# jaeyoungjo99/ELiMaLoc

Measured on AMD Instinct MI355X. Metric: ICP registrations/sec, 128k-pt scan vs 10M-pt map; pose err vs CPU ref, higher is better.
Workload: dtype f64

## Files before the change

elimaloc_amd/csrc/elm_api.cpp:

```cpp
#include <dlfcn.h>
#include <hip/hip_runtime.h>
#include <math.h>
#include <stdio.h>
#include <stdlib.h>
#include <string.h>
#include <unistd.h>

#include <algorithm>
#include <array>
#include <chrono>
#include <map>
#include <mutex>
#include <new>
#include <set>
#include <string>
#include <thread>
#include <vector>

#include "elm_hostapi.hpp"
#include "elm_internal.hpp"
#include "elm_la.hpp"

using namespace elm;

// ... 63 lines not shown
    int device = 0;
    uint64_t id = 0;
    hipStream_t stream = nullptr;
    hipStream_t copy_stream = nullptr, order_stream = nullptr, poll_stream = nullptr;
    hipEvent_t ev_iter[4] = {nullptr, nullptr, nullptr, nullptr};
    std::vector<hipEvent_t> ev_groups;
    uint16_t* d_hilbert = nullptr;
    DevBuf d_order_jobs, d_order_tmp, d_arena, d_raw, d_flagged, d_asym;
    DevBuf d_q0, d_q1, d_q2, d_q3, d_q4, d_q5;
    DevBuf d_reloc[16];
    bool work_counters = false;
    void* h_jobs = nullptr;
    size_t h_jobs_cap = 0;
    std::string last_error;
    DevBuf d_scans, d_state, d_partials, d_sums, d_T0, d_trace, d_stage_pts, d_active, d_queue, d_ds;
    int stream_hint_count = 0, stream_hint_slots = 0, stream_hint_iters = 0;
    int* h_active = nullptr;
    int iter_hint = 0;
    int iter_ring[8] = {0, 0, 0, 0, 0, 0, 0, 0};
    unsigned iter_ring_pos = 0;
    const void* iter_key_map = nullptr;
    int iter_key_method = -1, iter_key_batch = 0;
    void* h_state = nullptr;
    size_t h_state_cap = 0;
    void* h_trace = nullptr;
    size_t h_trace_cap = 0;
    void* h_stage = nullptr;
    size_t h_stage_cap = 0;
    std::vector<uint32_t> h_key, h_ord, h_tmp;
    std::vector<struct elm_scan*> scan_free;
// ... 169 lines not shown
    }
    {
        std::lock_guard<std::mutex> lk(g_live_mu);
        if (!g_live_ctx.erase(ctx)) return;
    }
    (void)hipSetDevice(ctx->device);
    if (ctx->stream) (void)hipStreamSynchronize(ctx->stream);
    if (ctx->comm && g_rccl.comm_destroy) g_rccl.comm_destroy(ctx->comm);
    for (hipStream_t st : {ctx->copy_stream, ctx->order_stream, ctx->poll_stream})
        if (st) { (void)hipStreamSynchronize(st); (void)hipStreamDestroy(st); }
    for (hipEvent_t e : {ctx->ev_iter[0], ctx->ev_iter[1], ctx->ev_iter[2], ctx->ev_iter[3]})
        if (e) (void)hipEventDestroy(e);
    for (hipEvent_t e : ctx->ev_groups) (void)hipEventDestroy(e);
    if (ctx->d_hilbert) (void)hipFree(ctx->d_hilbert);
    if (ctx->h_jobs) (void)hipHostFree(ctx->h_jobs);
    DevBuf* bufs[] = {&ctx->d_scans, &ctx->d_state, &ctx->d_partials, &ctx->d_sums, &ctx->d_T0, &ctx->d_trace, &ctx->d_stage_pts, &ctx->d_active, &ctx->d_queue, &ctx->d_ds,
                      &ctx->d_order_jobs, &ctx->d_order_tmp, &ctx->d_arena, &ctx->d_raw, &ctx->d_flagged, &ctx->d_asym, &ctx->d_q0, &ctx->d_q1, &ctx->d_q2, &ctx->d_q3, &ctx->d_q4, &ctx->d_q5};
    if (ctx->h_active) (void)hipHostFree(ctx->h_active);
    for (DevBuf* b : bufs)
        if (b->p) (void)hipFree(b->p);
    for (DevBuf& b : ctx->d_reloc)
        if (b.p) (void)hipFree(b.p);
    for (auto& b : ctx->scan_pool) (void)hipFree(b.first);
    for (elm_scan* f : ctx->scan_free) delete f;
    if (ctx->h_state) (void)hipHostFree(ctx->h_state);
    if (ctx->h_trace) (void)hipHostFree(ctx->h_trace);
    if (ctx->h_stage) (void)hipHostFree(ctx->h_stage);
    if (ctx->h_desc) (void)hipHostFree(ctx->h_desc);
    for (hipEvent_t e : ctx->events) (void)hipEventDestroy(e);
    if (ctx->stream) (void)hipStreamDestroy(ctx->stream);
    delete ctx;
// ... 1922 lines not shown
        q.hd[s].blk_begin = cap_blocks * (uint32_t)s; q.hd[s].blk_end = cap_blocks * (uint32_t)(s + 1);
    }
    elm_iter_trace* d_trace = nullptr;
    if (trace && (rc = reserve_trace(ctx, count, &d_trace)) != ELM_OK) return rc;
    HIPCHK(ctx, hipMemcpyAsync(q.d_q, q.hq, q.ctrl_off + sizeof(StreamCtrl), hipMemcpyHostToDevice, ctx->stream));
    HIPCHK(ctx, hipMemcpyAsync(ctx->d_scans.p, q.hd, (size_t)S * sizeof(ScanDesc), hipMemcpyHostToDevice, ctx->stream));
    HIPCHK(ctx, hipMemsetAsync(ctx->d_active.p, 0, 2 * sizeof(int), ctx->stream));
    if ((rc = set_reg_params(ctx, cfg, pc, blocks, S, cap_blocks)) != ELM_OK) return rc;
    const RegParams& rp = ctx->rp;

    ScanState* st = (ScanState*)ctx->d_state.p;
    ScanDesc* dsc = (ScanDesc*)ctx->d_scans.p;
    int* d_active = (int*)ctx->d_active.p;
    const bool distributed = (ctx->comm != nullptr) || (ctx->hook != nullptr);
    (void)hipGetLastError();
    launch_stream_refill(ctx->stream, dsc, st, S, q.d_q, q.d_qT0, q.d_out, q.d_ctrl, 1);
    ctx->events_used = 0;
    const int hard_limit = ((count + S - 1) / S + 1) * cfg->max_iteration;
    const bool same_shape = ctx->stream_hint_count == count && ctx->stream_hint_slots == S;
    const int predicted = same_shape ? ctx->stream_hint_iters : 0;
    double* const partials = (double*)ctx->d_partials.p;
    double* const sums = (double*)ctx->d_sums.p;
    int it = 0;
    for (; it < hard_limit; ++it) {
        if ((rc = enqueue_accumulate(ctx, map, dsc, S, blocks, st, rp, pc, partials)) != ELM_OK) return rc;
        if (distributed) {
            launch_solve(ctx->stream, dsc, S, st, partials, sums, rp, d_trace, 1, d_active);
            if ((rc = exchange(ctx, sums, (size_t)S * (rp.asym ? kSums + kAsymRecord : kSums))) != ELM_OK) return rc;
            const StreamArgs sv = {dsc, q.d_q, q.d_qT0, q.d_out, q.d_ctrl, 0,  1, 0, it};
            launch_solve(ctx->stream, dsc, S, st, partials, sums, rp, d_trace, 2, d_active, &sv);
            launch_stream_refill(ctx->stream, dsc, st, S, q.d_q, q.d_qT0, q.d_out, q.d_ctrl, 0,  0);
        } else {
            const StreamArgs sa = {dsc, q.d_q, q.d_qT0, q.d_out, q.d_ctrl, 0, 0, 0, it};
            launch_solve(ctx->stream, dsc, S, st, partials, sums, rp, d_trace, 0, d_active, &sa);
        }
        const int done_iters = it + 1;
        const bool look = predicted > 0 ? done_iters >= predicted : (done_iters >= (count + S - 1) / S && (done_iters % 2) == 0);
        if (look) {
            HIPCHK(ctx, hipMemcpyAsync(ctx->h_active, &q.d_ctrl->completed, sizeof(int), hipMemcpyDeviceToHost, ctx->stream));
            HIPCHK(ctx, hipStreamSynchronize(ctx->stream));
            if (*ctx->h_active == count) { ++it; break; }
        }
    }
    if ((rc = prof_mark(ctx)) != ELM_OK) return rc;
    HIPCHK(ctx, hipGetLastError());
    HIPCHK(ctx, hipMemcpyAsync(ctx->h_state, q.d_out, (size_t)count * sizeof(ScanState), hipMemcpyDeviceToHost, ctx->stream));
    if (trace) HIPCHK(ctx, hipMemcpyAsync(ctx->h_trace, ctx->d_trace.p, trace_bytes(count), hipMemcpyDeviceToHost, ctx->stream));
    ctx->h_active[2] = 0;
// ... 843 lines not shown
```

elimaloc_amd/csrc/elm_dev_pairs.hpp:

```cpp
#pragma once
#include <float.h>
#include <hip/hip_runtime.h>

#include "elm_internal.hpp"
#include "elm_la.hpp"

namespace elm {




__device__ __forceinline__ unsigned xcd_remap(unsigned bid, unsigned nb) {
    unsigned q = nb >> 3, r = nb & 7u, xcd = bid & 7u, idx = bid >> 3;
    return (xcd < r ? xcd * (q + 1) : r * (q + 1) + (xcd - r) * q) + idx;
}

struct Probe {
    int vid;
    unsigned start, cnt;
};
__device__ __forceinline__ Probe probe_voxel(const DevMap& m, int kx, int ky, int kz) {
    unsigned h = hash3(kx, ky, kz) & m.mask;
    Probe p;
    p.vid = -1;
// ... 371 lines not shown
    if (!(dfin < rp.th2)) return;
    if (bvid < 0) bmx = bmy = bmz = 0.0;
    voxel_pair<ELM_VGICP, ASSIGN>(acc, m, S, rp, gx, gy, gz, bvid, bmx, bmy, bmz);
}

__device__ __forceinline__ int find_scan(const ScanDesc* __restrict__ scans, int batch, unsigned L, const RegParams& rp) {
    if (rp.uniform_blocks) return (int)(L / rp.uniform_blocks);
    int lo = 0, hi = batch - 1;
    while (lo < hi) {
        const int mid = (lo + hi + 1) >> 1;
        if (scans[mid].blk_begin <= L) lo = mid; else hi = mid - 1;
    }
    return lo;
}

__device__ __forceinline__ void block_reduce_store(double* acc, double (*red)[32], double* __restrict__ out) {
    const int lane = threadIdx.x & 63, wave = threadIdx.x >> 6;
#pragma unroll
    for (int k = 0; k < 32; ++k) {
        const double v = wave_sum(acc[k]);
        if (lane == 0) red[wave][k] = v;
    }
    __syncthreads();
    if (threadIdx.x < 32)
        out[threadIdx.x] = ((red[0][threadIdx.x] + red[1][threadIdx.x]) + red[2][threadIdx.x]) + red[3][threadIdx.x];
}


__device__ __forceinline__ void publish_and_reduce(double value, unsigned L, int, unsigned, unsigned, double* __restrict__ partials, const RegParams&, double*) {
    if (threadIdx.x < (unsigned)kSums) partials[(size_t)L * kSums + threadIdx.x] = value;
// ... 13 lines not shown
```

elimaloc_amd/csrc/elm_internal.hpp:

```cpp
#pragma once
#include <hip/hip_runtime.h>
#include <stdint.h>

#include "../../include/elimaloc_hip.h"

namespace elm {

struct __attribute__((aligned(32))) HashSlot {
    int32_t kx, ky, kz;
    int32_t vid;
    uint32_t start;
    uint32_t cnt;
    uint32_t pad0, pad1;
};

struct __attribute__((packed, aligned(4))) Pt3 {
    float x, y, z;
};

struct __attribute__((aligned(16))) GridBlk {
    float x[4], y[4], z[4];
};

struct __attribute__((aligned(64))) VoxRec {
// ... 108 lines not shown
    int32_t total;
    int32_t ready;
    int32_t done_iter;
};

struct StreamArgs {
    ScanDesc* scans;
    const QueueItem* queue;
    const double* qT0;
    ScanState* out_state;
    StreamCtrl* ctrl;
    int32_t hostfed;
    int32_t save_only;
    int32_t stride;
    int32_t iter;
};

struct RegParams {
    double th;
    double th2;
    double lm_lambda;
    double term_thr;
    double min_overlap;
    double max_fitness;
    int32_t method;
    int32_t max_iter;
    uint32_t uniform_blocks;
    int32_t radar;
    int32_t _reserved0;
    int32_t stats;
    uint32_t* flagged;
    int32_t rank_check;
    int32_t _pad_rc;
    double* asym;
    double* asym_sums;
    double radar_var[3];
    const double* query;
    int32_t* q_out;
};
constexpr int kAsymRecord = 16;
constexpr int kRadarRecord = 64;

constexpr int kTileShift = 3, kTile = 1 << kTileShift;
constexpr int kBlock = 256;
constexpr int kInitPack = 8;
struct InitPack {
    ScanDesc d[kInitPack];
    double T0[kInitPack][16];
};
constexpr int kSums = ELM_PACKED_SUMS;

void launch_init_state(hipStream_t s, ScanState* st, const double* T0, int batch, int map_empty, int* active);
void launch_init_pack(hipStream_t s, ScanDesc* scans, ScanState* st, const InitPack& pack, int batch, int map_empty, int* active, const unsigned* n_dev);
void launch_stream_refill(hipStream_t s, ScanDesc* scans, ScanState* st, int slots, const QueueItem* queue, const double* qT0,
                          ScanState* out_state, StreamCtrl* ctrl, int first, int save = 1);
void launch_accumulate_radar(hipStream_t s, const DevMap& m, const ScanDesc* scans, int batch, int total_blocks, ScanState* st, double* partials,
                             const RegParams& rp);
void launch_accumulate_direct(hipStream_t s, const DevMap& m, const ScanDesc* scans, int batch, int total_blocks,
                              ScanState* st, double* partials, const RegParams& rp);
void launch_solve(hipStream_t s, const ScanDesc* scans, int batch, ScanState* st, const double* partials,
                  double* sums, const RegParams& rp, elm_iter_trace* trace, int mode, int* active, const StreamArgs* refill = nullptr);
void launch_nbr_count(hipStream_t s, const DevMap& m, const int32_t* qkeys, uint32_t n_q, uint32_t* counts, uint32_t* nocc);
void launch_accumulate_vnbr(hipStream_t s, const DevMap& m, const ScanDesc* scans, int batch, int total_blocks,
                            ScanState* st, double* partials, const RegParams& rp);
void launch_vnbr_fill(hipStream_t s, const DevMap& m, const int32_t* qkeys, uint32_t n_q, const uint32_t* offsets, VoxBlk* out_blk);
void launch_vox_rec_fill(hipStream_t s, const DevMap& m, VoxRec* out);
void launch_vface(hipStream_t s, const DevMap& m, const uint32_t* offsets, const uint32_t* counts, uint32_t n_q, uint32_t* face_cnt,
                  const uint32_t* face_off, VoxRec* out, int plain);
void launch_accumulate_cell(hipStream_t s, const DevMap& m, const ScanDesc* scans, int batch, int total_blocks,
                            ScanState* st, double* partials, const RegParams& rp);
// ... 135 lines not shown
```

elimaloc_amd/csrc/elm_k_cell.hip:

```cpp
#include <float.h>
#include <algorithm>
#include <hip/hip_runtime.h>

#include "elm_internal.hpp"
#include "elm_la.hpp"
#include "elm_dev_grid.hpp"

namespace elm {

template <int METHOD>
__global__ __launch_bounds__(kBlock, (METHOD == ELM_P2P ? kCellWaves : kCellWaves - 1)) void k_accumulate_cell(const DevMap m, const ScanDesc* __restrict__ scans, int batch,
                                                                            unsigned total_blocks, const ScanState* __restrict__ st,
                                                                            double* __restrict__ partials, const RegParams rp) {
    constexpr int NV = (METHOD == ELM_P2P) ? kP2PVals : kSums;
    __shared__ double s_buf[kRedPass * kBlock];
    __shared__ double s_red[kSums];
    __shared__ int s_res[kBlock];
    __shared__ int s_tst[kBlock];
    __shared__ unsigned s_cnt[kBlock / 64];
    __shared__ double s_asym[(METHOD == ELM_GICP) ? kAsymSums : 1];
    __shared__ unsigned s_hitw[kBlock / 64];
    PairSum PA;
    pair_sum_zero(PA);
    static_assert(sizeof(HardRec) * kBlock <= sizeof(double) * kRedPass * kBlock, "HardRec queue must fit the reduction buffer");
    const unsigned L = xcd_remap(blockIdx.x, total_blocks);
    const int s = find_scan(scans, batch, L, rp);
    const ScanState& S = st[s];
    if (S.done) return;
    const ScanDesc sd = scans[s];
    if (L >= sd.blk_end) return;
    const unsigned i = (L - sd.blk_begin) * kBlock + threadIdx.x;
    const bool valid = i < sd.n;
    double v[NV];
#pragma unroll
    for (int k = 0; k < NV; ++k) v[k] = 0.0;
    double px = 0.0, py = 0.0, pz = 0.0, gx = 0.0, gy = 0.0, gz = 0.0;
    QProbe qp;
    qp.start = 0; qp.cnt = 0; qp.nocc = 0; qp.qid = -1;
    int bj = -1;
    int n_tested = 0;
    float hr2 = __builtin_inff();
// ... 242 lines not shown
```

elimaloc_amd/csrc/elm_k_grid.hip:

```cpp
#include <float.h>
#include <algorithm>
#include <hip/hip_runtime.h>

#include "elm_internal.hpp"
#include "elm_la.hpp"
#include "elm_dev_grid.hpp"

namespace elm {

template <int METHOD, int COMPACT, int TILED, int STATS, int WIDE>
__global__ __launch_bounds__(kBlock, (METHOD == ELM_P2P ? (STATS ? 7 : kGridWaves) : kGicpWaves)) void k_accumulate_grid(
       const DevMap m, const ScanDesc* __restrict__ scans, int batch,
                                                                            unsigned total_blocks, const ScanState* __restrict__ st,
                                                                            double* __restrict__ partials, const RegParams rp) {
    constexpr int kStats = (STATS == 1) ? 1 : 0;
    constexpr bool QUERY = STATS == 2;
    constexpr int NV = (METHOD == ELM_P2P) ? (kStats ? kP2PVals : kP2PVals - 3) : kSums;
    __shared__ double s_buf[kRedPass * kBlock];
    __shared__ double s_red[kSums];
    __shared__ int s_res[kBlock];
    __shared__ int s_tst[kStats ? kBlock : 1];
    __shared__ float s_pz[METHOD == ELM_P2P ? kBlock : 1];
    __shared__ unsigned s_st[kStats ? kBlock : 1];
    __shared__ unsigned s_cnt[kBlock / 64];
    const unsigned L = xcd_remap(blockIdx.x, total_blocks);
    const int s = find_scan(scans, batch, L, rp);
    const ScanState& S = st[s];
    if (S.done) return;
    const ScanDesc sd = scans[s];
    if (L >= sd.blk_end) return;
    const unsigned i = (L - sd.blk_begin) * kBlock + threadIdx.x;
    const bool valid = i < sd.n;
    double v[(METHOD == ELM_P2P) ? NV : 1];
#pragma unroll
    for (int k = 0; k < ((METHOD == ELM_P2P) ? NV : 1); ++k) v[k] = 0.0;
    PairSum P;
    if (METHOD != ELM_P2P) pair_sum_zero(P);
    int bj = -1;
    int n_tested = 0;
    float hr2 = __builtin_inff();
    bool hard = false;
// ... 343 lines not shown
```

elimaloc_amd/csrc/elm_k_solve.hip:

```cpp
#include <float.h>
#include <algorithm>
#include <hip/hip_runtime.h>

#include "elm_internal.hpp"
#include "elm_la.hpp"
#include "elm_dev_reduce.hpp"

namespace elm {

__device__ void update_inverse(ScanState& S) {
    double R[9];
    for (int r = 0; r < 3; ++r)
        for (int c = 0; c < 3; ++c) R[r * 3 + c] = S.T[c * 4 + r];
    inv3(R, S.Rinv);
    for (int r = 0; r < 3; ++r)
        S.tinv[r] = -((S.Rinv[r * 3] * S.T[12] + S.Rinv[r * 3 + 1] * S.T[13]) + S.Rinv[r * 3 + 2] * S.T[14]);
}

__device__ void init_scan_state(ScanState& S, const double* __restrict__ T0, int reg, int map_empty) {
    for (int k = 0; k < 16; ++k) S.T[k] = T0[k];
    update_inverse(S);
    S.fitness = 0.0;
    for (int k = 0; k < 36; ++k) S.local_cov[k] = (k % 7 == 0) ? 1.0 : 0.0;
    S.n_corr_last = 0.0;
// ... 22 lines not shown
    ScanDesc d = pack.d[s];
    if (n_dev) {
        d.n = *n_dev;
        d.n_total = d.n;
        d.blk_end = d.blk_begin + (d.n + kBlock - 1) / kBlock;
    }
    scans[s] = d;
    init_scan_state(st[s], pack.T0[s], s, map_empty);
}
void launch_init_pack(hipStream_t s, ScanDesc* scans, ScanState* st, const InitPack& pack, int batch, int map_empty, int* active, const unsigned* n_dev) {
    hipLaunchKernelGGL(k_init_pack, dim3(1), dim3(64), 0, s, scans, st, pack, batch, map_empty, active, n_dev);
}

constexpr int kMaxSlots = 4096;
__global__ __launch_bounds__(1024) void k_stream_refill(ScanDesc* scans, ScanState* st, int slots, const QueueItem* __restrict__ queue,
                                                       const double* __restrict__ qT0, ScanState* out_state, StreamCtrl* ctrl, int first, int save) {
    __shared__ int s_assign[kMaxSlots];
    __shared__ int s_save[kMaxSlots];
    for (int s = threadIdx.x; s < slots; s += blockDim.x) s_save[s] = (!first && st[s].done && st[s].reg >= 0) ? st[s].reg : -1;
    __syncthreads();
    {
        __shared__ int s_wtot[16];
        const int per = (slots + (int)blockDim.x - 1) / (int)blockDim.x, s0 = (int)threadIdx.x * per, s1 = min(slots, s0 + per);
        int mine = 0;
        for (int s = s0; s < s1; ++s) mine += (first || s_save[s] >= 0) ? 1 : 0;
        int inc = mine;
#pragma unroll
        for (int off = 1; off < 64; off <<= 1) {
            const int o = __shfl_up(inc, off, 64);
            if ((int)(threadIdx.x & 63u) >= off) inc += o;
        }
// ... 28 lines not shown
        for (int k = (int)(threadIdx.x & 63); k < W; k += 64) dst[k] = src[k];
    }
    __syncthreads();
    for (int s = threadIdx.x; s < slots; s += blockDim.x) {
        const int r = s_assign[s];
        if (r >= 0) {
            const QueueItem q = queue[r];
            scans[s].pts = q.pts;
            scans[s].n = q.n;
            scans[s].n_total = q.n_total;
            init_scan_state(st[s], qT0 + (size_t)r * 16, r, 0);
        } else if (r == -2) {
            st[s].done = 1;
            st[s].reg = -1;
        }
    }
}

__device__ __forceinline__ void wave_ldlt6(double a, const double* b, double x[6], bool want_inv, double& inv_elem) {
    const int lane = threadIdx.x & 63;
    const int li = (lane < 36) ? lane / 6 : 0, lj = (lane < 36) ? lane % 6 : 0;
    unsigned active = 0x3Fu;
    int order[6];
    double piv[6];
    int rank_i = 6, rank_j = 6, rank_l = 6;
    double d0[6];
    int pos[6];
#pragma unroll
    for (int i = 0; i < 6; ++i) { d0[i] = fabs(__shfl(a, i * 7, 64)); pos[i] = i; }
    auto d0_of = [&](int r) { return r == 0 ? d0[0] : r == 1 ? d0[1] : r == 2 ? d0[2] : r == 3 ? d0[3] : r == 4 ? d0[4] : d0[5]; };
#pragma unroll
// ... 144 lines not shown
        return (r < sa.ctrl->total) ? r : -1;
    }
    if (!sa.hostfed) {
        const int r = atomicAdd(&sa.ctrl->next, 1);
        return (r < sa.ctrl->total) ? r : -1;
    }
    int old = __hip_atomic_load(&sa.ctrl->next, __ATOMIC_RELAXED, __HIP_MEMORY_SCOPE_AGENT);
    for (;;) {
        const int ready = __hip_atomic_load(&sa.ctrl->ready, __ATOMIC_RELAXED, __HIP_MEMORY_SCOPE_SYSTEM);
        if (old >= ready) return -1;
        const int seen = atomicCAS(&sa.ctrl->next, old, old + 1);
        if (seen == old) return old;
        old = seen;
    }
}
__device__ __forceinline__ void start_slot(const StreamArgs& sa, ScanState& S, int s, int prev) {
    const int lane = threadIdx.x & 63;
    int r = 0;
    if (lane == 0) r = claim_registration(sa, prev);
    r = __shfl(r, 0, 64);
    if (r >= 0) {
        const double* T0 = sa.qT0 + (size_t)r * 16;
        if (lane >= 1 && lane < 37) S.local_cov[lane - 1] = ((lane - 1) % 7 == 0) ? 1.0 : 0.0;
        if (lane == 0) {
            const QueueItem q = sa.queue[r];
            sa.scans[s].pts = q.pts;
            sa.scans[s].n = q.n;
            sa.scans[s].n_total = q.n_total;
            for (int k = 0; k < 16; ++k) S.T[k] = T0[k];
            update_inverse(S);
            S.fitness = 0.0;
            S.n_corr_last = 0.0;
            S.pt_iters = 0.0; S.cand_total = 0.0; S.occ_total = 0.0; S.fallback_blocks = 0.0; S.tested_total = 0.0;
            S.done = 0;
            S.success = 0;
            S.gate = 0;
            S.iters = 0;
            S.reg = r;
            S._pad = 0;
        }
    } else if (lane == 0) {
        S.done = 1;
        S.reg = -1;
    }
}
__device__ __forceinline__ void finish_slot(const StreamArgs& sa, ScanState& S, int s) {
#if !defined(__gfx950__) && !defined(__gfx942__) && !defined(__gfx90a__) && defined(__HIP_DEVICE_COMPILE__)
#error "finish_slot relies on gfx9 memory ordering (one vmcnt for loads and stores, write-through vector L1)"
#endif
    constexpr int W = (int)(sizeof(ScanState) / sizeof(double));
    const int lane = threadIdx.x & 63;
    __builtin_amdgcn_fence(__ATOMIC_RELEASE, "workgroup");
    __builtin_amdgcn_s_waitcnt(0);
    __builtin_amdgcn_wave_barrier();
    __builtin_amdgcn_fence(__ATOMIC_ACQUIRE, "workgroup");
    const int reg_old = __hip_atomic_load(&S.reg, __ATOMIC_RELAXED, __HIP_MEMORY_SCOPE_AGENT);
    const double* src = reinterpret_cast<const double*>(&S);
    double* dst = reinterpret_cast<double*>(&sa.out_state[reg_old]);
    for (int k = lane; k < W; k += 64) dst[k] = __hip_atomic_load(src + k, __ATOMIC_RELAXED, __HIP_MEMORY_SCOPE_AGENT);
    if (lane == 0 && atomicAdd(&sa.ctrl->completed, 1) + 1 == sa.ctrl->total) sa.ctrl->done_iter = sa.iter;
    __builtin_amdgcn_fence(__ATOMIC_RELEASE, "workgroup");
    __builtin_amdgcn_s_waitcnt(0);
    __builtin_amdgcn_wave_barrier();
    if (sa.save_only) return;
    start_slot(sa, S, s, reg_old);
}

constexpr int kSolveThreads = 1024;
__device__ __forceinline__ double rank_check_id(int reg, int iters) {
    return 16.0 * (double)((reg < 0 ? -1 : (reg & 0x7FFFF)) + 1) + (double)(iters & 15);
}
template <int NT>
__global__ __launch_bounds__(NT, 1) void k_solve(const ScanDesc* scans, ScanState* st,
                                                         const double* __restrict__ partials, double* sums,
                                                         const RegParams rp, elm_iter_trace* trace, int mode, int* active,
                                                         const StreamArgs sa) {
    const int s = blockIdx.x;
    ScanState& S = st[s];
    const int t = threadIdx.x;
    __shared__ double tot[kSums];
    __shared__ double part[kSolveThreads / 32][kSums];
    static_assert(NT == kSolveThreads, "solve workgroup size");
    const bool done = S.done != 0;
    const bool radar = rp.radar != 0;
    __shared__ double full[36];
    const bool asym = rp.asym != nullptr && !radar && rp.method != ELM_P2P;
    __shared__ double dsum[kAsymSums];
    __shared__ double apart[kSolveThreads / kAsymSums][kAsymSums];
    if (radar) {
        double a = 0.0;
        if (mode != 2) {
            const int k = t & 63, g = t >> 6;
            double* part64 = &part[0][0];
            double v = 0.0;
            if (!done) {
                const ScanDesc sd = scans[s];
                for (unsigned b = sd.blk_begin + g; b < sd.blk_end; b += kSolveThreads / 64) v += partials[(size_t)b * kRadarSums + k];
            }
            part64[g * 64 + k] = v;
            __syncthreads();
            if (t < 64) {
                a = part64[t];
#pragma unroll
                for (int q = 1; q < kSolveThreads / 64; ++q) a += part64[q * 64 + t];
                if (mode == 1) sums[(size_t)s * kRadarSums + t] = (t < kRadarAcc) ? a : 0.0;
            }
            if (mode == 1) return;
        } else if (t < 64) {
            a = sums[(size_t)s * kRadarSums + t];
        }
        if (t < 64) {
            if (t < 36) full[t] = a;
            else if (t < kRadarAcc) tot[21 + (t - 36)] = a;
        }
    } else if (mode != 2) {
        const int k = t & 31;
        constexpr unsigned G = kSolveThreads / 32;
        auto group_sum = [&](int g) -> double {
            double v = 0.0;
            if (!done) {
                const ScanDesc sd = scans[s];
                unsigned b = sd.blk_begin + g;
                double v0 = 0.0, v1 = 0.0, v2 = 0.0, v3 = 0.0;
                for (; b + 15 * G < sd.blk_end; b += 16 * G) {
                    double a[16];
#pragma unroll
                    for (int q = 0; q < 16; ++q) a[q] = partials[(size_t)(b + q * G) * kSums + k];
#pragma unroll
                    for (int q = 0; q < 16; q += 4) { v0 += a[q]; v1 += a[q + 1]; v2 += a[q + 2]; v3 += a[q + 3]; }
                }
                for (; b + 3 * G < sd.blk_end; b += 4 * G) {
                    const double a0 = partials[(size_t)b * kSums + k], a1 = partials[(size_t)(b + G) * kSums + k];
                    const double a2 = partials[(size_t)(b + 2 * G) * kSums + k], a3 = partials[(size_t)(b + 3 * G) * kSums + k];
                    v0 += a0; v1 += a1; v2 += a2; v3 += a3;
                }
                if (b < sd.blk_end) { v0 += partials[(size_t)b * kSums + k]; b += G; }
// ... 3 lines not shown
            }
            return v;
        };
        if (NT == kSolveThreads) {
            part[t >> 5][k] = group_sum(t >> 5);
        } else {
#pragma unroll 1
            for (int g = t >> 5; g < (int)G; g += NT / 32) part[g][k] = group_sum(g);
        }
        if (asym) {
            constexpr int GA = kSolveThreads / kAsymSums;
            const int k2 = t & (kAsymSums - 1);
            auto side_sum = [&](int g) -> double {
                double v = 0.0;
                if (!done) {
                    const ScanDesc sd = scans[s];
                    for (unsigned b = sd.blk_begin + (unsigned)g; b < sd.blk_end; b += (unsigned)GA) v += rp.asym[(size_t)b * kAsymSums + k2];
                }
                return v;
            };
            if (NT == kSolveThreads) {
                apart[t / kAsymSums][k2] = side_sum(t / kAsymSums);
            } else {
#pragma unroll 1
                for (int g = t / kAsymSums; g < GA; g += NT / kAsymSums) apart[g][k2] = side_sum(g);
            }
        }
        __syncthreads();
        if (t < 32) {
            double a = part[0][t];
#pragma unroll
// ... 59 lines not shown
                double row = 0.0;
                for (int l = 0; l < 3; ++l) row += hw[(bi + k) * 6 + (bj + l)] * S.T[jj * 4 + l];
                h += S.T[ii * 4 + k] * row;
            }
            if (i <= j) tot[tri(i, j)] = h;
            if (nonsym) full[t] = h;
        }
        if (t < 6) {
            const int bi = (t / 3) * 3, ii = t % 3;
            tot[21 + t] = (S.T[ii * 4 + 0] * bw[bi] + S.T[ii * 4 + 1] * bw[bi + 1]) + S.T[ii * 4 + 2] * bw[bi + 2];
        }
        __builtin_amdgcn_s_waitcnt(0);
        __builtin_amdgcn_wave_barrier();
    }

    const ScanDesc sd = scans[s];
    const int iter = S.iters + 1;
    const double n_corr = tot[28];
    if (lead) {
        S.iters = iter;
        S.n_corr_last = n_corr;
        S.pt_iters += (double)sd.n_total;
        S.cand_total += tot[29];
        S.occ_total += tot[30];
        const double fb = floor(tot[31] / 1099511627776.0);
        S.fallback_blocks += fb;
        S.tested_total += tot[31] - fb * 1099511627776.0;
    }
    elm_iter_trace* tr = (trace && iter <= ELM_MAX_ITER_TRACE) ? &trace[(size_t)S.reg * ELM_MAX_ITER_TRACE + (iter - 1)] : nullptr;

    const float ratio_f = (float)n_corr / (float)sd.n_total;
    if ((double)ratio_f < rp.min_overlap) {
        if (lead) {
            if (tr) {
                for (int k = 0; k < 36; ++k) tr->JTJ[k] = 0.0;
                for (int k = 0; k < 6; ++k) { tr->JTr[k] = 0.0; tr->x[k] = 0.0; }
                tr->residual_sum = tot[27];
                tr->n_corr = n_corr;
                tr->step_norm = 0.0;
                for (int k = 0; k < 16; ++k) tr->T[k] = S.T[k];
            }
            S.done = 1;
            atomicSub(active, 1);
            S.success = 0;
            S.gate = 2;
        }
        if (sa.ctrl) finish_slot(sa, S, s);
        return;
    }
    const double fitness = tot[27] / n_corr;

    const int li = (t < 36) ? t / 6 : 0, lj = (t < 36) ? t % 6 : 0;
    const bool full36 = radar || nonsym;
    const double hij = full36 ? full[(li < lj ? lj : li) * 6 + (li < lj ? li : lj)] : tot[tri(li < lj ? li : lj, li < lj ? lj : li)];
    const double a = (li == lj) ? hij + rp.lm_lambda * hij : hij;
    double x[6], inv_elem;
    wave_ldlt6(a, &tot[21], x, rp.method == ELM_GICP && !full36, inv_elem);
    if (rp.method == ELM_GICP && !full36 && t < 36) S.local_cov[t] = inv_elem;
    if (rp.method == ELM_GICP && full36) {
        const double el = (t < 36) ? ((li == lj) ? full[t] + rp.lm_lambda * full[t] : full[t]) : 0.0;
        const double inv_el = wave_inverse6_partial_piv(el);
        const double inv_t = __shfl(inv_el, lj * 6 + li, 64);
// ... 20 lines not shown
            for (int k = 0; k < 6; ++k) { tr->JTr[k] = tot[21 + k]; tr->x[k] = x[k]; }
            tr->residual_sum = tot[27];
            tr->n_corr = n_corr;
            tr->step_norm = step;
            for (int k = 0; k < 16; ++k) tr->T[k] = Tn[k];
        }
        if (step < rp.term_thr || iter >= rp.max_iter) {
            S.done = 1;
            atomicSub(active, 1);
            const bool bad = fitness > rp.max_fitness;
            S.success = bad ? 0 : 1;
            S.gate = bad ? 3 : 0;
            fin = true;
        }
    }
    if (sa.ctrl && __shfl((int)fin, 0, 64)) finish_slot(sa, S, s);
}

__device__ __forceinline__ void smallest_eigenvector3(const double C[9], double n[3]) {
    double A[9] = {C[0], C[3], C[6], C[3], C[4], C[7], C[6], C[7], C[8]};
    double V[9] = {1, 0, 0, 0, 1, 0, 0, 0, 1};
    for (int sweep = 0; sweep < 60; ++sweep) {
        const double off = fabs(A[3]) + fabs(A[6]) + fabs(A[7]);
        if (off == 0.0) break;
        for (int p = 0; p < 2; ++p)
            for (int q = p + 1; q < 3; ++q) {
                if (A[p * 3 + q] == 0.0) continue;
                const double theta = (A[q * 3 + q] - A[p * 3 + p]) / (2.0 * A[p * 3 + q]);
                const double t = (theta >= 0 ? 1.0 : -1.0) / (fabs(theta) + sqrt(theta * theta + 1.0));
                const double c = 1.0 / sqrt(t * t + 1.0), s = t * c;
                for (int k = 0; k < 3; ++k) { const double akp = A[k * 3 + p], akq = A[k * 3 + q]; A[k * 3 + p] = c * akp - s * akq; A[k * 3 + q] = s * akp + c * akq; }
// ... 93 lines not shown

__global__ void k_slots_idle(ScanDesc* scans, ScanState* st, int slots, unsigned cap_blocks) {
    const int s = blockIdx.x * blockDim.x + threadIdx.x;
    if (s >= slots) return;
    scans[s].pts = nullptr; scans[s].n = 0; scans[s].n_total = 0;
    scans[s].blk_begin = cap_blocks * (unsigned)s; scans[s].blk_end = cap_blocks * (unsigned)(s + 1);
    st[s].done = 1;
    st[s].reg = -1;
}

__global__ void k_publish_ready(StreamCtrl* ctrl, int ready) {
    __hip_atomic_store(&ctrl->ready, ready, __ATOMIC_RELAXED, __HIP_MEMORY_SCOPE_SYSTEM);
}

void launch_stream_refill(hipStream_t s, ScanDesc* scans, ScanState* st, int slots, const QueueItem* queue, const double* qT0,
                          ScanState* out_state, StreamCtrl* ctrl, int first, int save) {
    hipLaunchKernelGGL(k_stream_refill, dim3(1), dim3(1024), 0, s, scans, st, slots, queue, qT0, out_state, ctrl, first, save);
}

void launch_init_state(hipStream_t s, ScanState* st, const double* T0, int batch, int map_empty, int* active) {
    hipLaunchKernelGGL(k_init_state, dim3((batch + 63) / 64), dim3(64), 0, s, st, T0, batch, map_empty, active);
}

void launch_solve(hipStream_t s, const ScanDesc* scans, int batch, ScanState* st, const double* partials,
                  double* sums, const RegParams& rp, elm_iter_trace* trace, int mode, int* active, const StreamArgs* refill) {
    StreamArgs sa = {nullptr, nullptr, nullptr, nullptr, nullptr, 0, 0, 0, 0};
    if (refill) sa = *refill;
    const int threads = mode == 2 ? 64 : kSolveThreads;
    hipLaunchKernelGGL(k_solve<kSolveThreads>, dim3(batch), dim3(threads), 0, s, scans, st, partials, sums, rp, trace, mode, active, sa);
}

void launch_publish_ready(hipStream_t s, StreamCtrl* ctrl, int ready) { hipLaunchKernelGGL(k_publish_ready, dim3(1), dim3(1), 0, s, ctrl, ready); }

void launch_slots_idle(hipStream_t s, ScanDesc* scans, ScanState* st, int slots, unsigned cap_blocks) {
    hipLaunchKernelGGL(k_slots_idle, dim3((slots + 255) / 256), dim3(256), 0, s, scans, st, slots, cap_blocks);
}

int stream_max_slots() { return kMaxSlots; }

}
```

elimaloc_amd/csrc/elm_k_vnbr.hip:

```cpp
#include <float.h>
#include <algorithm>
#include <hip/hip_runtime.h>

#include "elm_internal.hpp"
#include "elm_la.hpp"
#include "elm_dev_grid.hpp"

namespace elm {


constexpr int kVnbrRecs = 3;
constexpr int kAvgRecs = 1;
constexpr int kVnbrBlks = 1;
constexpr int kVnbrWaves = 1;
template <int METHOD, int COMPACT, int STATS, int FACES>
__global__ __launch_bounds__(kBlock, kVnbrWaves) void k_accumulate_vnbr(const DevMap m, const ScanDesc* __restrict__ scans, int batch,
                                                            unsigned total_blocks, const ScanState* __restrict__ st,
                                                            double* __restrict__ partials, const RegParams rp) {
    constexpr int kStats = (STATS == 1) ? 1 : 0;
    constexpr bool QUERY = STATS == 2;
    __shared__ double s_buf[kRedPass * kBlock];
    __shared__ double s_red[kSums];
    const unsigned L = xcd_remap(blockIdx.x, total_blocks);
    const int s = find_scan(scans, batch, L, rp);
    const ScanState& S = st[s];
    if (S.done) return;
    const ScanDesc sd = scans[s];
    if (L >= sd.blk_end) return;
    const unsigned i = (L - sd.blk_begin) * kBlock + threadIdx.x;
    const bool valid = i < sd.n;
    if (FACES == 3) {
        if (rp.flagged[L] == 0u) return;
        __syncthreads();
        if (threadIdx.x == 0) rp.flagged[L] = 0u;
    }
    PairSum P;
    pair_sum_zero(P);
    if (valid) {
        double px = 0.0, py = 0.0, pz = 0.0, gx, gy, gz;
// ... 294 lines not shown
```

elimaloc_amd/csrc/elm_k_walk.hip:

```cpp
#include <float.h>
#include <algorithm>
#include <hip/hip_runtime.h>

#include "elm_internal.hpp"
#include "elm_la.hpp"
#include "elm_dev_pairs.hpp"

namespace elm {

template <int METHOD>
__global__ __launch_bounds__(kBlock) void k_accumulate_direct(const DevMap m, const ScanDesc* __restrict__ scans,
                                                              int batch, unsigned total_blocks,
                                                              const ScanState* __restrict__ st,
                                                              double* __restrict__ partials, const RegParams rp) {
    const unsigned L = xcd_remap(blockIdx.x, total_blocks);
    const int s = find_scan(scans, batch, L, rp);
    const ScanState& S = st[s];
    if (S.done) return;
    const ScanDesc sd = scans[s];
    if (L >= sd.blk_end) return;
    const unsigned i = (L - sd.blk_begin) * kBlock + threadIdx.x;
    const bool valid = i < sd.n;
    double acc[32];
#pragma unroll
    for (int k = 0; k < 32; ++k) acc[k] = 0.0;
    if (valid) {
        const Pt3 pf = sd.pts[i];
        const double px = pf.x, py = pf.y, pz = pf.z;
        const double gx = ((S.T[0] * px + S.T[4] * py) + S.T[8] * pz) + S.T[12];
        const double gy = ((S.T[1] * px + S.T[5] * py) + S.T[9] * pz) + S.T[13];
        const double gz = ((S.T[2] * px + S.T[6] * py) + S.T[10] * pz) + S.T[14];
// ... 37 lines not shown
        const int lane = threadIdx.x & 63, wave = threadIdx.x >> 6;
#pragma unroll
        for (int k = 0; k < 32; ++k) {
            const double v = wave_sum(acc[k]);
            if (lane == 0) red[wave][k] = v;
        }
        __syncthreads();
        if (threadIdx.x < 32) sum = ((red[0][threadIdx.x] + red[1][threadIdx.x]) + red[2][threadIdx.x]) + red[3][threadIdx.x];
    }
    publish_and_reduce(sum, L, s, sd.blk_begin, sd.blk_end, partials, rp, s_scr);
}

template <int METHOD>
__global__ __launch_bounds__(kBlock) void k_accumulate_radar(const DevMap m, const ScanDesc* __restrict__ scans, int batch, unsigned total_blocks,
                                                             const ScanState* __restrict__ st, double* __restrict__ partials, const RegParams rp) {
    const unsigned L = xcd_remap(blockIdx.x, total_blocks);
    const int s = find_scan(scans, batch, L, rp);
    const ScanState& S = st[s];
    if (S.done) return;
    const ScanDesc sd = scans[s];
    if (L >= sd.blk_end) return;
    const unsigned i = (L - sd.blk_begin) * kBlock + threadIdx.x;
    double acc[kRadarAcc];
#pragma unroll
    for (int k = 0; k < kRadarAcc; ++k) acc[k] = 0.0;
    if (i < sd.n) {
        const Pt3 pf = sd.pts[i];
        const double px = pf.x, py = pf.y, pz = pf.z;
        const double gx = ((S.T[0] * px + S.T[4] * py) + S.T[8] * pz) + S.T[12];
        const double gy = ((S.T[1] * px + S.T[5] * py) + S.T[9] * pz) + S.T[13];
        const double gz = ((S.T[2] * px + S.T[6] * py) + S.T[10] * pz) + S.T[14];
        double Cs[9] = {1, 0, 0, 0, 1, 0, 0, 0, 1};
// ... 146 lines not shown
```

Measured before the change: 98430.

## Compact accumulate grid onto a device-maintained live-slot list

```diff
diff --git a/elimaloc_amd/csrc/elm_api.cpp b/elimaloc_amd/csrc/elm_api.cpp
--- a/elimaloc_amd/csrc/elm_api.cpp
+++ b/elimaloc_amd/csrc/elm_api.cpp
@@ -101,6 +101,7 @@
     size_t h_jobs_cap = 0;
     std::string last_error;
     DevBuf d_scans, d_state, d_partials, d_sums, d_T0, d_trace, d_stage_pts, d_active, d_queue, d_ds;
+    DevBuf d_live;
     int stream_hint_count = 0, stream_hint_slots = 0, stream_hint_iters = 0;
     int* h_active = nullptr;
     int iter_hint = 0;
@@ -300,7 +301,7 @@
     for (hipEvent_t e : ctx->ev_groups) (void)hipEventDestroy(e);
     if (ctx->d_hilbert) (void)hipFree(ctx->d_hilbert);
     if (ctx->h_jobs) (void)hipHostFree(ctx->h_jobs);
-    DevBuf* bufs[] = {&ctx->d_scans, &ctx->d_state, &ctx->d_partials, &ctx->d_sums, &ctx->d_T0, &ctx->d_trace, &ctx->d_stage_pts, &ctx->d_active, &ctx->d_queue, &ctx->d_ds,
+    DevBuf* bufs[] = {&ctx->d_scans, &ctx->d_state, &ctx->d_partials, &ctx->d_sums, &ctx->d_T0, &ctx->d_trace, &ctx->d_stage_pts, &ctx->d_active, &ctx->d_queue, &ctx->d_ds, &ctx->d_live,
                       &ctx->d_order_jobs, &ctx->d_order_tmp, &ctx->d_arena, &ctx->d_raw, &ctx->d_flagged, &ctx->d_asym, &ctx->d_q0, &ctx->d_q1, &ctx->d_q2, &ctx->d_q3, &ctx->d_q4, &ctx->d_q5};
     if (ctx->h_active) (void)hipHostFree(ctx->h_active);
     for (DevBuf* b : bufs)
@@ -2253,7 +2254,12 @@
     int* d_active = (int*)ctx->d_active.p;
     const bool distributed = (ctx->comm != nullptr) || (ctx->hook != nullptr);
     (void)hipGetLastError();
-    launch_stream_refill(ctx->stream, dsc, st, S, q.d_q, q.d_qT0, q.d_out, q.d_ctrl, 1);
+    int* d_live = nullptr;
+    if (!distributed && cap_blocks > 0) {
+        if ((rc = dev_reserve(ctx, ctx->d_live, (size_t)(kLiveHead + 2 * S) * sizeof(int))) != ELM_OK) return rc;
+        d_live = (int*)ctx->d_live.p;
+    }
+    launch_stream_refill(ctx->stream, dsc, st, S, q.d_q, q.d_qT0, q.d_out, q.d_ctrl, 1, 1, d_live);
     ctx->events_used = 0;
     const int hard_limit = ((count + S - 1) / S + 1) * cfg->max_iteration;
     const bool same_shape = ctx->stream_hint_count == count && ctx->stream_hint_slots == S;
@@ -2262,7 +2268,9 @@
     double* const sums = (double*)ctx->d_sums.p;
     int it = 0;
     for (; it < hard_limit; ++it) {
-        if ((rc = enqueue_accumulate(ctx, map, dsc, S, blocks, st, rp, pc, partials)) != ELM_OK) return rc;
+        RegParams rpi = rp;
+        if (d_live) { rpi.live_count = d_live + ((it + 1) & 1); rpi.live = d_live + kLiveHead + ((it + 1) & 1) * S; }
+        if ((rc = enqueue_accumulate(ctx, map, dsc, S, blocks, st, rpi, pc, partials)) != ELM_OK) return rc;
         if (distributed) {
             launch_solve(ctx->stream, dsc, S, st, partials, sums, rp, d_trace, 1, d_active);
             if ((rc = exchange(ctx, sums, (size_t)S * (rp.asym ? kSums + kAsymRecord : kSums))) != ELM_OK) return rc;
@@ -2270,7 +2278,8 @@
             launch_solve(ctx->stream, dsc, S, st, partials, sums, rp, d_trace, 2, d_active, &sv);
             launch_stream_refill(ctx->stream, dsc, st, S, q.d_q, q.d_qT0, q.d_out, q.d_ctrl, 0,  0);
         } else {
-            const StreamArgs sa = {dsc, q.d_q, q.d_qT0, q.d_out, q.d_ctrl, 0, 0, 0, it};
+            StreamArgs sa = {dsc, q.d_q, q.d_qT0, q.d_out, q.d_ctrl, 0, 0, 0, it};
+            if (d_live) { sa.live_out = d_live + kLiveHead + (it & 1) * S; sa.live_out_count = d_live + (it & 1); sa.live_zero = d_live + ((it + 1) & 1); }
             launch_solve(ctx->stream, dsc, S, st, partials, sums, rp, d_trace, 0, d_active, &sa);
         }
         const int done_iters = it + 1;
diff --git a/elimaloc_amd/csrc/elm_dev_pairs.hpp b/elimaloc_amd/csrc/elm_dev_pairs.hpp
--- a/elimaloc_amd/csrc/elm_dev_pairs.hpp
+++ b/elimaloc_amd/csrc/elm_dev_pairs.hpp
@@ -409,6 +409,20 @@
     return lo;
 }
 
+__device__ __forceinline__ bool block_to_scan(const ScanDesc* __restrict__ scans, int batch, unsigned total_blocks, const RegParams& rp, unsigned& L, int& s) {
+    if (rp.live) {
+        const unsigned ub = rp.uniform_blocks, nb = (unsigned)*rp.live_count * ub, bid = blockIdx.x;
+        if ((bid >> 3) >= (nb >> 3) + (((bid & 7u) < (nb & 7u)) ? 1u : 0u)) return false;
+        const unsigned Lv = xcd_remap(bid, nb), q = Lv / ub;
+        s = rp.live[q];
+        L = (unsigned)s * ub + (Lv - q * ub);
+        return true;
+    }
+    L = xcd_remap(blockIdx.x, total_blocks);
+    s = find_scan(scans, batch, L, rp);
+    return true;
+}
+
 __device__ __forceinline__ void block_reduce_store(double* acc, double (*red)[32], double* __restrict__ out) {
     const int lane = threadIdx.x & 63, wave = threadIdx.x >> 6;
 #pragma unroll
diff --git a/elimaloc_amd/csrc/elm_internal.hpp b/elimaloc_amd/csrc/elm_internal.hpp
--- a/elimaloc_amd/csrc/elm_internal.hpp
+++ b/elimaloc_amd/csrc/elm_internal.hpp
@@ -146,7 +146,11 @@
     int32_t save_only;
     int32_t stride;
     int32_t iter;
-};
+    int32_t* live_out;
+    int32_t* live_out_count;
+    int32_t* live_zero;
+};
+constexpr int kLiveHead = 16;
 
 struct RegParams {
     double th;
@@ -169,6 +173,8 @@
     double radar_var[3];
     const double* query;
     int32_t* q_out;
+    const int32_t* live;
+    const int32_t* live_count;
 };
 constexpr int kAsymRecord = 16;
 constexpr int kRadarRecord = 64;
@@ -185,7 +191,8 @@
 void launch_init_state(hipStream_t s, ScanState* st, const double* T0, int batch, int map_empty, int* active);
 void launch_init_pack(hipStream_t s, ScanDesc* scans, ScanState* st, const InitPack& pack, int batch, int map_empty, int* active, const unsigned* n_dev);
 void launch_stream_refill(hipStream_t s, ScanDesc* scans, ScanState* st, int slots, const QueueItem* queue, const double* qT0,
-                          ScanState* out_state, StreamCtrl* ctrl, int first, int save = 1);
+                          ScanState* out_state, StreamCtrl* ctrl, int first, int save = 1,
+                          int* live_head = nullptr);
 void launch_accumulate_radar(hipStream_t s, const DevMap& m, const ScanDesc* scans, int batch, int total_blocks, ScanState* st, double* partials,
                              const RegParams& rp);
 void launch_accumulate_direct(hipStream_t s, const DevMap& m, const ScanDesc* scans, int batch, int total_blocks,
diff --git a/elimaloc_amd/csrc/elm_k_cell.hip b/elimaloc_amd/csrc/elm_k_cell.hip
--- a/elimaloc_amd/csrc/elm_k_cell.hip
+++ b/elimaloc_amd/csrc/elm_k_cell.hip
@@ -23,8 +23,9 @@
     PairSum PA;
     pair_sum_zero(PA);
     static_assert(sizeof(HardRec) * kBlock <= sizeof(double) * kRedPass * kBlock, "HardRec queue must fit the reduction buffer");
-    const unsigned L = xcd_remap(blockIdx.x, total_blocks);
-    const int s = find_scan(scans, batch, L, rp);
+    unsigned L;
+    int s;
+    if (!block_to_scan(scans, batch, total_blocks, rp, L, s)) return;
     const ScanState& S = st[s];
     if (S.done) return;
     const ScanDesc sd = scans[s];
diff --git a/elimaloc_amd/csrc/elm_k_grid.hip b/elimaloc_amd/csrc/elm_k_grid.hip
--- a/elimaloc_amd/csrc/elm_k_grid.hip
+++ b/elimaloc_amd/csrc/elm_k_grid.hip
@@ -23,8 +23,9 @@
     __shared__ float s_pz[METHOD == ELM_P2P ? kBlock : 1];
     __shared__ unsigned s_st[kStats ? kBlock : 1];
     __shared__ unsigned s_cnt[kBlock / 64];
-    const unsigned L = xcd_remap(blockIdx.x, total_blocks);
-    const int s = find_scan(scans, batch, L, rp);
+    unsigned L;
+    int s;
+    if (!block_to_scan(scans, batch, total_blocks, rp, L, s)) return;
     const ScanState& S = st[s];
     if (S.done) return;
     const ScanDesc sd = scans[s];
diff --git a/elimaloc_amd/csrc/elm_k_solve.hip b/elimaloc_amd/csrc/elm_k_solve.hip
--- a/elimaloc_amd/csrc/elm_k_solve.hip
+++ b/elimaloc_amd/csrc/elm_k_solve.hip
@@ -60,7 +60,8 @@
 
 constexpr int kMaxSlots = 4096;
 __global__ __launch_bounds__(1024) void k_stream_refill(ScanDesc* scans, ScanState* st, int slots, const QueueItem* __restrict__ queue,
-                                                       const double* __restrict__ qT0, ScanState* out_state, StreamCtrl* ctrl, int first, int save) {
+                                                       const double* __restrict__ qT0, ScanState* out_state, StreamCtrl* ctrl, int first, int save,
+                                                       int* live_head) {
     __shared__ int s_assign[kMaxSlots];
     __shared__ int s_save[kMaxSlots];
     for (int s = threadIdx.x; s < slots; s += blockDim.x) s_save[s] = (!first && st[s].done && st[s].reg >= 0) ? st[s].reg : -1;
@@ -119,7 +120,9 @@
             st[s].done = 1;
             st[s].reg = -1;
         }
-    }
+        if (first && live_head) live_head[kLiveHead + slots + s] = s;
+    }
+    if (first && live_head && threadIdx.x == 0) { live_head[0] = 0; live_head[1] = slots; }
 }
 
 __device__ __forceinline__ void wave_ldlt6(double a, const double* b, double x[6], bool want_inv, double& inv_elem) {
@@ -294,20 +297,15 @@
         old = seen;
     }
 }
-__device__ __forceinline__ void start_slot(const StreamArgs& sa, ScanState& S, int s, int prev) {
+__device__ __forceinline__ bool start_slot_claimed(const StreamArgs& sa, ScanState& S, int s, int r, const QueueItem& q, const double* T0v) {
     const int lane = threadIdx.x & 63;
-    int r = 0;
-    if (lane == 0) r = claim_registration(sa, prev);
-    r = __shfl(r, 0, 64);
     if (r >= 0) {
-        const double* T0 = sa.qT0 + (size_t)r * 16;
         if (lane >= 1 && lane < 37) S.local_cov[lane - 1] = ((lane - 1) % 7 == 0) ? 1.0 : 0.0;
         if (lane == 0) {
-            const QueueItem q = sa.queue[r];
             sa.scans[s].pts = q.pts;
             sa.scans[s].n = q.n;
             sa.scans[s].n_total = q.n_total;
-            for (int k = 0; k < 16; ++k) S.T[k] = T0[k];
+            for (int k = 0; k < 16; ++k) S.T[k] = T0v[k];
             update_inverse(S);
             S.fitness = 0.0;
             S.n_corr_last = 0.0;
@@ -323,27 +321,53 @@
         S.done = 1;
         S.reg = -1;
     }
-}
-__device__ __forceinline__ void finish_slot(const StreamArgs& sa, ScanState& S, int s) {
+    return r >= 0;
+}
+__device__ __forceinline__ void fetch_registration(const StreamArgs& sa, int r, QueueItem& q, double* T0v) {
+    q = sa.queue[r];
+    const double* T0 = sa.qT0 + (size_t)r * 16;
+#pragma unroll
+    for (int k = 0; k < 16; ++k) T0v[k] = T0[k];
+}
+__device__ __forceinline__ bool start_slot(const StreamArgs& sa, ScanState& S, int s, int prev) {
+    const int lane = threadIdx.x & 63;
+    int r = 0;
+    if (lane == 0) r = claim_registration(sa, prev);
+    r = __shfl(r, 0, 64);
+    QueueItem q = {nullptr, 0, 0};
+    double T0v[16];
+    if (lane == 0 && r >= 0) fetch_registration(sa, r, q, T0v);
+    return start_slot_claimed(sa, S, s, r, q, T0v);
+}
+__device__ __forceinline__ bool finish_slot(const StreamArgs& sa, ScanState& S, int s) {
 #if !defined(__gfx950__) && !defined(__gfx942__) && !defined(__gfx90a__) && defined(__HIP_DEVICE_COMPILE__)
 #error "finish_slot relies on gfx9 memory ordering (one vmcnt for loads and stores, write-through vector L1)"
 #endif
     constexpr int W = (int)(sizeof(ScanState) / sizeof(double));
     const int lane = threadIdx.x & 63;
+    int r = -1;
+    if (!sa.save_only && lane == 0) r = claim_registration(sa, S.reg);
     __builtin_amdgcn_fence(__ATOMIC_RELEASE, "workgroup");
     __builtin_amdgcn_s_waitcnt(0);
     __builtin_amdgcn_wave_barrier();
     __builtin_amdgcn_fence(__ATOMIC_ACQUIRE, "workgroup");
+    r = __shfl(r, 0, 64);
+    QueueItem q = {nullptr, 0, 0};
+    double T0v[16];
+    if (lane == 0 && r >= 0) fetch_registration(sa, r, q, T0v);
     const int reg_old = __hip_atomic_load(&S.reg, __ATOMIC_RELAXED, __HIP_MEMORY_SCOPE_AGENT);
     const double* src = reinterpret_cast<const double*>(&S);
     double* dst = reinterpret_cast<double*>(&sa.out_state[reg_old]);
+    int n_done = 0;
+    if (lane == 0) n_done = atomicAdd(&sa.ctrl->completed, 1) + 1;
     for (int k = lane; k < W; k += 64) dst[k] = __hip_atomic_load(src + k, __ATOMIC_RELAXED, __HIP_MEMORY_SCOPE_AGENT);
-    if (lane == 0 && atomicAdd(&sa.ctrl->completed, 1) + 1 == sa.ctrl->total) sa.ctrl->done_iter = sa.iter;
-    __builtin_amdgcn_fence(__ATOMIC_RELEASE, "workgroup");
-    __builtin_amdgcn_s_waitcnt(0);
     __builtin_amdgcn_wave_barrier();
-    if (sa.save_only) return;
-    start_slot(sa, S, s, reg_old);
+    const bool on = sa.save_only ? false : start_slot_claimed(sa, S, s, r, q, T0v);
+    if (lane == 0 && n_done == sa.ctrl->total) sa.ctrl->done_iter = sa.iter;
+    return on;
+}
+__device__ __forceinline__ void live_append(const StreamArgs& sa, int s) {
+    if (sa.live_out && (threadIdx.x & 63u) == 0u) sa.live_out[atomicAdd(sa.live_out_count, 1)] = s;
 }
 
 constexpr int kSolveThreads = 1024;
@@ -361,7 +385,9 @@
     __shared__ double tot[kSums];
     __shared__ double part[kSolveThreads / 32][kSums];
     static_assert(NT == kSolveThreads, "solve workgroup size");
+    const ScanDesc sd = scans[s];
     const bool done = S.done != 0;
+    if (sa.live_zero && s == 0 && t == 0) *sa.live_zero = 0;
     const bool radar = rp.radar != 0;
     __shared__ double full[36];
     const bool asym = rp.asym != nullptr && !radar && rp.method != ELM_P2P;
@@ -374,7 +400,6 @@
             double* part64 = &part[0][0];
             double v = 0.0;
             if (!done) {
-                const ScanDesc sd = scans[s];
                 for (unsigned b = sd.blk_begin + g; b < sd.blk_end; b += kSolveThreads / 64) v += partials[(size_t)b * kRadarSums + k];
             }
             part64[g * 64 + k] = v;
@@ -399,7 +424,6 @@
         auto group_sum = [&](int g) -> double {
             double v = 0.0;
             if (!done) {
-                const ScanDesc sd = scans[s];
                 unsigned b = sd.blk_begin + g;
                 double v0 = 0.0, v1 = 0.0, v2 = 0.0, v3 = 0.0;
                 for (; b + 15 * G < sd.blk_end; b += 16 * G) {
@@ -433,7 +457,6 @@
             auto side_sum = [&](int g) -> double {
                 double v = 0.0;
                 if (!done) {
-                    const ScanDesc sd = scans[s];
                     for (unsigned b = sd.blk_begin + (unsigned)g; b < sd.blk_end; b += (unsigned)GA) v += rp.asym[(size_t)b * kAsymSums + k2];
                 }
                 return v;
@@ -523,7 +546,6 @@
         __builtin_amdgcn_wave_barrier();
     }
 
-    const ScanDesc sd = scans[s];
     const int iter = S.iters + 1;
     const double n_corr = tot[28];
     if (lead) {
@@ -554,7 +576,8 @@
             S.success = 0;
             S.gate = 2;
         }
-        if (sa.ctrl) finish_slot(sa, S, s);
+        const bool on = sa.ctrl ? finish_slot(sa, S, s) : false;
+        if (on) live_append(sa, s);
         return;
     }
     const double fitness = tot[27] / n_corr;
@@ -605,7 +628,9 @@
             fin = true;
         }
     }
-    if (sa.ctrl && __shfl((int)fin, 0, 64)) finish_slot(sa, S, s);
+    const bool finished = __shfl((int)fin, 0, 64) != 0;
+    const bool on = finished ? (sa.ctrl ? finish_slot(sa, S, s) : false) : true;
+    if (on) live_append(sa, s);
 }
 
 __device__ __forceinline__ void smallest_eigenvector3(const double C[9], double n[3]) {
@@ -729,8 +754,8 @@
 }
 
 void launch_stream_refill(hipStream_t s, ScanDesc* scans, ScanState* st, int slots, const QueueItem* queue, const double* qT0,
-                          ScanState* out_state, StreamCtrl* ctrl, int first, int save) {
-    hipLaunchKernelGGL(k_stream_refill, dim3(1), dim3(1024), 0, s, scans, st, slots, queue, qT0, out_state, ctrl, first, save);
+                          ScanState* out_state, StreamCtrl* ctrl, int first, int save, int* live_head) {
+    hipLaunchKernelGGL(k_stream_refill, dim3(1), dim3(1024), 0, s, scans, st, slots, queue, qT0, out_state, ctrl, first, save, live_head);
 }
 
 void launch_init_state(hipStream_t s, ScanState* st, const double* T0, int batch, int map_empty, int* active) {
@@ -739,7 +764,7 @@
 
 void launch_solve(hipStream_t s, const ScanDesc* scans, int batch, ScanState* st, const double* partials,
                   double* sums, const RegParams& rp, elm_iter_trace* trace, int mode, int* active, const StreamArgs* refill) {
-    StreamArgs sa = {nullptr, nullptr, nullptr, nullptr, nullptr, 0, 0, 0, 0};
+    StreamArgs sa = {nullptr, nullptr, nullptr, nullptr, nullptr, 0, 0, 0, 0, nullptr, nullptr, nullptr};
     if (refill) sa = *refill;
     const int threads = mode == 2 ? 64 : kSolveThreads;
     hipLaunchKernelGGL(k_solve<kSolveThreads>, dim3(batch), dim3(threads), 0, s, scans, st, partials, sums, rp, trace, mode, active, sa);
diff --git a/elimaloc_amd/csrc/elm_k_vnbr.hip b/elimaloc_amd/csrc/elm_k_vnbr.hip
--- a/elimaloc_amd/csrc/elm_k_vnbr.hip
+++ b/elimaloc_amd/csrc/elm_k_vnbr.hip
@@ -21,8 +21,9 @@
     constexpr bool QUERY = STATS == 2;
     __shared__ double s_buf[kRedPass * kBlock];
     __shared__ double s_red[kSums];
-    const unsigned L = xcd_remap(blockIdx.x, total_blocks);
-    const int s = find_scan(scans, batch, L, rp);
+    unsigned L;
+    int s;
+    if (!block_to_scan(scans, batch, total_blocks, rp, L, s)) return;
     const ScanState& S = st[s];
     if (S.done) return;
     const ScanDesc sd = scans[s];
diff --git a/elimaloc_amd/csrc/elm_k_walk.hip b/elimaloc_amd/csrc/elm_k_walk.hip
--- a/elimaloc_amd/csrc/elm_k_walk.hip
+++ b/elimaloc_amd/csrc/elm_k_walk.hip
@@ -13,8 +13,9 @@
                                                               int batch, unsigned total_blocks,
                                                               const ScanState* __restrict__ st,
                                                               double* __restrict__ partials, const RegParams rp) {
-    const unsigned L = xcd_remap(blockIdx.x, total_blocks);
-    const int s = find_scan(scans, batch, L, rp);
+    unsigned L;
+    int s;
+    if (!block_to_scan(scans, batch, total_blocks, rp, L, s)) return;
     const ScanState& S = st[s];
     if (S.done) return;
     const ScanDesc sd = scans[s];
@@ -82,8 +83,9 @@
 template <int METHOD>
 __global__ __launch_bounds__(kBlock) void k_accumulate_radar(const DevMap m, const ScanDesc* __restrict__ scans, int batch, unsigned total_blocks,
                                                              const ScanState* __restrict__ st, double* __restrict__ partials, const RegParams rp) {
-    const unsigned L = xcd_remap(blockIdx.x, total_blocks);
-    const int s = find_scan(scans, batch, L, rp);
+    unsigned L;
+    int s;
+    if (!block_to_scan(scans, batch, total_blocks, rp, L, s)) return;
     const ScanState& S = st[s];
     if (S.done) return;
     const ScanDesc sd = scans[s];
```

Result: slower. 93580 (-4.9%).
